# ming71/rotate-yolov3

Hardware: AMD Instinct MI355X
Metric: images/sec fwd+bwd at 608^2 (train step, backend=hip) (higher is better)
Workload: dtype bf16; 1 GPU; configs[3]: Darknet-53 train step (fwd + riou loss + bwd + grad all-reduce + SGD), bs=64/GPU 608x608, synthetic HRSC-shaped targets; global_batch=64, parallelism=dp1, gradients=250 MB fp32 in 4 flat buckets, fp32 on the wire

## Files before the change

include/ryolo.h:

```cpp
#ifndef RYOLO_H
#define RYOLO_H

#include <stddef.h>
#include <stdint.h>

#ifdef __cplusplus
extern "C" {
#endif

#define RYOLO_OK 0
#define RYOLO_EINVAL -1
#define RYOLO_ELAUNCH -2
#define RYOLO_ETOOBIG -3

#define RYOLO_RNMS_MAX_BOXES 262144

const char *ryolo_strerror(int code);
int ryolo_abi_version(void);
const char *ryolo_build_id(void);
int ryolo_set_tuning(const char *name, const char *value);

size_t ryolo_rnms_workspace_bytes(int n);
int ryolo_rnms(const float *dets, int n, int row_stride, float thr, int64_t *keep_out, int32_t *num_keep,
               void *workspace, size_t workspace_bytes, void *stream);
// ... 114 lines not shown
int ryolo_conv_dgrad_tap_table(int ksize, int stride, int *host_out );
int ryolo_conv_pack_weights_dgrad(const float *w_oihw, int Cout, int Cin, int ksize, int stride, void *packed,
                                  const int *taps_table ,
                                  void *stream);
int ryolo_conv2d_dgrad(const ryolo_conv_desc *forward_desc, const void *dz, int dz_cstride, const void *packed_dgrad,
                       const float *ones, const float *zeros , void *dx, int accumulate, void *stream);
int ryolo_conv2d_dgrad_bnreduce_rows(const ryolo_conv_desc *forward_desc);
int ryolo_conv2d_dgrad_bnreduce(const ryolo_conv_desc *forward_desc, const void *dz, int dz_cstride, const void *packed_dgrad,
                                const float *ones, const float *zeros, void *dx, int accumulate,
                                const void *z , int z_cstride,
                                const float *scale, const float *shift, const float *mean, const float *invstd ,
                                const float *slope , float *part , void *stream);
int ryolo_bn_act_bwd_reduced(const void *z, int z_cstride, const void *dy, int dy_cstride, const float *scale, const float *shift,
                             const float *mean, const float *invstd, int act , const float *slope, void *dz,
                             int dz_cstride, long long npix, int C, float *dgamma, float *dbeta, float *dslope, const float *part,
                             int rows, void *workspace , size_t workspace_bytes, void *stream);
size_t ryolo_conv_wgrad_workspace_bytes(const ryolo_conv_desc *forward_desc);
int ryolo_conv2d_wgrad_partials(const ryolo_conv_desc *forward_desc, const void *x, const void *dz, int dz_cstride, int Cin_real,
                                float *grad_oihw, int accumulate, void *workspace, size_t workspace_bytes, void *stream);
int ryolo_conv2d_wgrad_reduce(const ryolo_conv_desc *forward_desc, const void *x, const void *dz, int dz_cstride, int Cin_real,
                              float *grad_oihw, int accumulate, void *workspace, size_t workspace_bytes, void *stream);

typedef struct ryolo_wgrad_reduce_job {
    const float *part;
    float *g;
    int S, Cout, Cin_real, Cin_k, ks, Kpad, Cout_pad, accumulate;
    int kind;
    int block_begin, block_end;
    int wide;
} ryolo_wgrad_reduce_job;
int ryolo_conv_wgrad_reduce_job_fill(ryolo_wgrad_reduce_job *host_job, const ryolo_conv_desc *forward_desc, int Cin_real, const void *workspace,
                                     float *grad_oihw, int accumulate);
int ryolo_conv_wgrad_reduce_batch(const ryolo_wgrad_reduce_job *device_jobs, int njobs, int total_blocks, void *stream);
int ryolo_conv2d_wgrad(const ryolo_conv_desc *forward_desc, const void *x, const void *dz, int dz_cstride, int Cin_real,
                       float *grad_oihw , int accumulate, void *workspace,
                       size_t workspace_bytes, void *stream);
int ryolo_upsample2x_bwd(const void *dy, int dy_cstride, void *dx, int dx_cstride, int N, int H, int W, int C,
                         int accumulate, void *stream);
int ryolo_pgrad_to_nhwc(const float *pgrad, int bs, int na, int ny, int nx, int no, void *out, int out_cstride,
                        void *stream);

typedef struct ryolo_pack_job {
    const void *src;
    void *dst;
    int kind, Cout, Cin, KS, Cin_pad, ntaps, Kpad, rows;
    int khs[9], kws[9];
    int block_begin, block_end;
} ryolo_pack_job;
int ryolo_conv_pack_job_fill(ryolo_pack_job *host_jobs, const float *w_oihw, int Cout, int Cin, int ksize, int stride,
                             int Cin_pad, void *packed_fwd, void *packed_dgrad);
int ryolo_conv_pack_batch(const ryolo_pack_job *device_jobs, int njobs, int total_blocks, void *stream);

#define RYOLO_MAX_HEADS 4
int ryolo_build_targets(const float *tpad, const unsigned char *valid, int NT, int nheads, int na, const float *const *ng,
                        const float *const *anchor_vec, float iou_t, float ang_t, float context_factor, float *const *w,
                        long long *const *idx, float *const *box, float *const *npos, void *stream);
size_t ryolo_yolo_loss_bitmap_bytes(long long cells);
int ryolo_yolo_loss(const float *p, int bs, int na, int ny, int nx, int no, int nc, const float *w, int NT,
                    const long long *b, const long long *gj, const long long *gi, const long long *cls, const float *txy,
                    const float *twh, const float *ta, const float *anchor_vec , const float *npos, float giou,
                    float reg_w, float cls_w, float cls_pw, float obj_w, float obj_pw,
                    int iou_mode ,
                    unsigned *bitmap, float *dp, float *items , void *stream);

int ryolo_yolo_loss_nhwc(const void *head, int head_cstride, const float *p, int bs, int na, int ny, int nx, int no, int nc,
                         const float *w, int NT, const long long *b, const long long *gj, const long long *gi,
// ... 38 lines not shown
```

rotate-yolov3_amd/csrc/rnms.hip:

```cpp
#include <hip/hip_runtime.h>
#include <hipcub/hipcub.hpp>
#include <stdint.h>

#include <mutex>

#include "../../include/ryolo.h"
#include "conv_common.h"

#pragma clang fp contract(off)

namespace {

constexpr int WAVE = 64;
constexpr int MAX_PTS = 24;
constexpr int FAST_PTS = 8;

__device__ __forceinline__ void sincosf_cr(float a, float &s_out, float &c_out) {
    double x = (double)a;
    if (!(fabs(x) <= 1.0e6)) {
        if (!(fabs(x) <= 3.5e38)) {
            s_out = (float)(x - x);
            c_out = (float)(x - x);
            return;
        }
// ... 787 lines not shown
static std::mutex g_side_mutex;
static SidePool g_side[16];
static SidePool *side_pool(hipStream_t stream) {
    int dev = 0;
    if (hipGetDevice(&dev) != hipSuccess || dev < 0 || dev >= 16) return nullptr;
    SidePool &sp = g_side[dev];
    if (sp.state == 0) {
        hipStreamCaptureStatus cs = hipStreamCaptureStatusNone;
        if (hipStreamIsCapturing(stream, &cs) != hipSuccess || cs != hipStreamCaptureStatusNone) { (void)hipGetLastError(); return nullptr; }
        const bool ok = hipStreamCreateWithFlags(&sp.s, hipStreamNonBlocking) == hipSuccess &&
                        hipEventCreateWithFlags(&sp.a, hipEventDisableTiming) == hipSuccess &&
                        hipEventCreateWithFlags(&sp.b, hipEventDisableTiming) == hipSuccess;
        if (!ok) (void)hipGetLastError();
        sp.state = ok ? 1 : -1;
    }
    return sp.state == 1 ? &sp : nullptr;
}
constexpr int SPLIT_MIN_ROWS = 320;

}

extern "C" {

const char *ryolo_strerror(int code) {
    switch (code) {
        case RYOLO_OK: return "ok";
        case RYOLO_EINVAL: return "invalid argument";
        case RYOLO_ELAUNCH: return "HIP launch failed (no gfx950 device, or a previous asynchronous error)";
        case RYOLO_ETOOBIG: return "too many boxes for one rotated-NMS call";
        default: return "unknown ryolo error";
    }
}

int ryolo_abi_version(void) { return 2; }

void ryolo_rnms_count_pairs(uint64_t *device_counter) { g_pair_counter = (unsigned long long *)device_counter; }


size_t ryolo_rnms_workspace_bytes(int n) {
    if (n <= 0) return 256;
    if (n > RYOLO_RNMS_MAX_BOXES) return 0;
    return rnms_layout(n).total;
}

int ryolo_rnms(const float *dets, int n, int row_stride, float thr, int64_t *keep_out, int32_t *num_keep,
               void *workspace, size_t workspace_bytes, void *stream_) {
    hipStream_t stream = (hipStream_t)stream_;
    if (n < 0 || !num_keep) return RYOLO_EINVAL;
    if (n == 0) {
        return hipMemsetAsync(num_keep, 0, sizeof(int32_t), stream) == hipSuccess ? RYOLO_OK : RYOLO_ELAUNCH;
    }
    if (!dets || !keep_out || !workspace || row_stride < 6) return RYOLO_EINVAL;
    if (n > RYOLO_RNMS_MAX_BOXES) return RYOLO_ETOOBIG;
    const RnmsLayout L = rnms_layout(n);
    if (workspace_bytes < L.total) return RYOLO_EINVAL;
    char *ws = (char *)workspace;
    uint32_t *keys_in = (uint32_t *)(ws + L.keys_in), *keys_out = (uint32_t *)(ws + L.keys_out);
    int32_t *idx_in = (int32_t *)(ws + L.idx_in), *order = (int32_t *)(ws + L.order);
    float4 *P0 = (float4 *)(ws + L.p0), *P1 = (float4 *)(ws + L.p1), *AUX = (float4 *)(ws + L.aux);
    uint4 *summ = (uint4 *)(ws + L.summ);
    unsigned char *flags = (unsigned char *)(ws + L.flags);
    unsigned long long *tiles = (unsigned long long *)(ws + L.tiles);

    const int tb = 256, nb = (n + tb - 1) / tb;
    hipLaunchKernelGGL(rnms_keys_kernel, dim3(nb), dim3(tb), 0, stream, dets, n, row_stride, keys_in, idx_in);
    size_t cub_bytes = L.cub_bytes;
    if (hipcub::DeviceRadixSort::SortPairs(ws + L.cub, cub_bytes, keys_in, keys_out, idx_in, order, n, 0, 32,
// ... 103 lines not shown
```

rotate-yolov3_amd/csrc/train.hip:

```cpp
#include <hip/hip_runtime.h>
#include <stdint.h>
#include <stdlib.h>

#include "../../include/ryolo.h"

namespace {

typedef __attribute__((ext_vector_type(8))) __bf16 bf16x8;
typedef __attribute__((ext_vector_type(4))) float f32x4;
typedef __attribute__((address_space(3))) void *lds_vp;
typedef short s16x4 __attribute__((ext_vector_type(4)));
typedef short s16x8 __attribute__((ext_vector_type(8)));

__device__ __forceinline__ s16x4 lds_read_tr16(const char *addr) {
#if defined(__HIP_DEVICE_COMPILE__)
    return __builtin_amdgcn_ds_read_tr16_b64_v4i16((__attribute__((address_space(3))) s16x4 *)(addr));
#else
    return s16x4{0, 0, 0, 0};
#endif
}

template <int T>
__device__ __forceinline__ int wg_swz(int row) {
    if (T >= 128) return (row & 3) | (((row >> 3) & 1) << 2);
// ... 139 lines not shown
#pragma unroll
        for (int ks = 0; ks < 2; ks++) {
            bf16x8 af[NF], bfr[NF];
#pragma unroll
            for (int f = 0; f < NF; f++) {
                const s16x4 a0 = lds_read_tr16(abuf + offa[f] + (ks * 32) * ROWB);
                const s16x4 a1 = lds_read_tr16(abuf + offa[f] + (ks * 32 + 4) * ROWB);
                const s16x4 b0 = lds_read_tr16(bbuf + offb[f] + (ks * 32) * ROWB);
                const s16x4 b1 = lds_read_tr16(bbuf + offb[f] + (ks * 32 + 4) * ROWB);
                af[f] = __builtin_bit_cast(bf16x8, __builtin_shufflevector(a0, a1, 0, 1, 2, 3, 4, 5, 6, 7));
                bfr[f] = __builtin_bit_cast(bf16x8, __builtin_shufflevector(b0, b1, 0, 1, 2, 3, 4, 5, 6, 7));
            }
#pragma unroll
            for (int a = 0; a < NF; a++)
#pragma unroll
                for (int c = 0; c < NF; c++)
                    acc[a][c] = __builtin_amdgcn_mfma_f32_16x16x32_bf16(af[a], bfr[c], acc[a][c], 0, 0, 0);
        }
    }
    float *out = p.part + (size_t)split * p.Cout_pad * p.Kpad;
#pragma unroll
    for (int a = 0; a < NF; a++)
#pragma unroll
        for (int c = 0; c < NF; c++)
#pragma unroll
            for (int r = 0; r < 4; r++) {
                const int co = co0 + wr * WT + a * 16 + kg * 4 + r;
                const int ci = ci0 + wc * WT + c * 16 + fr;
                if (co < p.Cout && ci < p.Cin) out[(size_t)co * p.Kpad + tap * p.Cin + ci] = acc[a][c][r];
            }
}

template <int TM, int TN, int ABL = 0, int NW = 4, int NT = 1>
__global__ void __launch_bounds__(NW * 64, NW == 8 ? (TM * TN > 256 * 128 ? 2 : 4) : 1) wgrad_wide_kernel(const WgradParams p) {
    constexpr int KPX = 32, NST = 3;
    constexpr int WM = TM / (NW / 2), WN = NT * TN / 2, NFA = WM / 16, NFB = WN / 16;
    constexpr int ROW_A = TM * 2, ROW_B = TN * 2;
    constexpr int TILE_A = KPX * ROW_A, TILE_B = KPX * ROW_B, STAGE = TILE_A + NT * TILE_B;
    constexpr int CH_A = TM / 8, CH_B = TN / 8;
    constexpr int PPP_A = 64 / CH_A, PPP_B = 64 / CH_B;
    constexpr int PPW_A = TILE_A / 1024 / NW, PPW_B = NT * TILE_B / 1024 / NW;
    constexpr int PPT_B = TILE_B / 1024;
    constexpr int NLD = PPW_A + PPW_B;
    static_assert(TM >= 64 && TN >= 64 && CH_A <= 64 && TILE_A % (1024 * NW) == 0 && (NT * TILE_B) % (1024 * NW) == 0, "tile shape");
    static_assert(NT == 1 || (NT * TN) % 32 == 0, "whole fragments per wave column");
    extern __shared__ __attribute__((aligned(16))) char smem[];

    const int tid = threadIdx.x, lane = tid & 63;
    const int wave = __builtin_amdgcn_readfirstlane(tid >> 6);
    int b = blockIdx.x;
    {
        const int per = gridDim.x >> 3;
        if (b < per * 8) b = (b & 7) * per + (b >> 3);
    }
    const int ci_t = b % p.ci_tiles; b /= p.ci_tiles;
    const int co_t = b % p.co_tiles; b /= p.co_tiles;
    const int ntg = (p.ks * p.ks) / NT;
    const int tap = (b % ntg) * NT; b /= ntg;
    const int split = b;
    const int kh = tap / p.ks, kw = tap % p.ks;
    const int co0 = co_t * TM, ci0 = ci_t * TN;
    const int pix_lo = split * p.chunk, pix_hi = min(p.M, pix_lo + p.chunk);

    int a_pix[PPW_A], a_col[PPW_A];
#pragma unroll
    for (int j = 0; j < PPW_A; j++) {
        const int tp = (wave * PPW_A + j) * PPP_A + lane / CH_A;
        a_pix[j] = tp;
        a_col[j] = (co0 + (((lane % CH_A) ^ (wg_swz<TM>(tp) << 1)) * 8)) * 2;
    }
    int b_pix[PPW_B], b_col[PPW_B], b_kw[PPW_B];
#pragma unroll
    for (int j = 0; j < PPW_B; j++) {
        const int q = wave * PPW_B + j;
        const int tp = (NT == 1 ? q : q % PPT_B) * PPP_B + lane / CH_B;
        b_pix[j] = tp;
        b_kw[j] = kw + (NT == 1 ? 0 : q / PPT_B);
        b_col[j] = (ci0 + (((lane % CH_B) ^ (wg_swz<TN>(tp) << 1)) * 8)) * 2;
    }

    const i32x4 rs_x = make_rsrc_words(p.x, p.x_bytes);
    const unsigned lds0 = (unsigned)(size_t)(__attribute__((address_space(3))) char *)smem;
    const unsigned a_step = (unsigned)(KPX * p.dz_cs * 2);
    unsigned long long a_base = (unsigned long long)p.dz + (unsigned long long)pix_lo * (unsigned long long)(p.dz_cs * 2);
    unsigned a_rec = (unsigned)((pix_hi - pix_lo) * p.dz_cs * 2);
    int a_vo[PPW_A];
#pragma unroll
    for (int j = 0; j < PPW_A; j++) a_vo[j] = a_pix[j] * p.dz_cs * 2 + a_col[j];
    const int x_cs2 = p.x_cs * 2;
    const int b_dw = KPX * p.stride, b_doff = KPX * p.stride * x_cs2;
    const int wi_wrap0 = p.Wo * p.stride - p.pad, hi_top = p.Ho * p.stride - p.pad + kh;
    const int b_wos = p.Wo * p.stride, b_hos = p.Ho * p.stride;
    const int b_rowjump = (p.stride * p.W - p.Wo * p.stride) * x_cs2, b_imgjump = (p.H - p.Ho * p.stride) * p.W * x_cs2;
    int b_rem = pix_hi - pix_lo;
    int b_hi[PPW_B], b_wi[PPW_B], b_off[PPW_B];
#pragma unroll
    for (int j = 0; j < PPW_B; j++) {
        const int pg = pix_lo + b_pix[j];
        const int wo = pg % p.Wo, t = pg / p.Wo;
        b_hi[j] = (t % p.Ho) * p.stride - p.pad + kh;
        b_wi[j] = wo * p.stride - p.pad + b_kw[j];
        b_off[j] = (int)(((long long)((t / p.Ho) * p.H + b_hi[j]) * p.W + b_wi[j]) * x_cs2) + b_col[j];
    }
    auto stage_a = [&](int buf, int j) __attribute__((always_inline)) {
        i32x4 r;
        r[0] = __builtin_amdgcn_readfirstlane((int)(unsigned)a_base);
        r[1] = __builtin_amdgcn_readfirstlane((int)(unsigned)(a_base >> 32));
        r[2] = __builtin_amdgcn_readfirstlane((int)a_rec);
        r[3] = 0x00020000;
        buffer_load_lds16_raw(r, lds0 + buf * STAGE + (wave * PPW_A + j) * 1024, a_vo[j]);
    };
    auto stage_b = [&](int buf, int j) __attribute__((always_inline)) {
        const bool ok = b_pix[j] < b_rem && (unsigned)b_hi[j] < (unsigned)p.H && (unsigned)b_wi[j] < (unsigned)p.W;
        buffer_load_lds16_raw(rs_x, lds0 + buf * STAGE + TILE_A + (wave * PPW_B + j) * 1024, ok ? b_off[j] : (int)0x80000000);
        b_wi[j] += b_dw;
        b_off[j] += b_doff;
        const int wi_wrap = wi_wrap0 + b_kw[j];
        auto wrap = [&]() __attribute__((always_inline)) {
// ... 65 lines not shown
        }
        __builtin_amdgcn_s_setprio(1);
#pragma unroll
        for (int a = 0; a < NFA; a++)
#pragma unroll
            for (int c = 0; c < NFB; c++)
                acc[a][c] = __builtin_amdgcn_mfma_f32_16x16x32_bf16(af[a], bfr[c], acc[a][c], 0, 0, 0);
        __builtin_amdgcn_s_setprio(0);
        cur = cur == NST - 1 ? 0 : cur + 1;
        nxt = nxt == NST - 1 ? 0 : nxt + 1;
    }
    asm volatile("s_waitcnt vmcnt(0)" ::: "memory");
    float *out = p.part + (size_t)split * p.Cout_pad * p.Kpad;
    if (ABL & 1) {
        float t = 0.f;
#pragma unroll
        for (int a = 0; a < NFA; a++)
#pragma unroll
            for (int c = 0; c < NFB; c++) t += acc[a][c][0] + acc[a][c][1] + acc[a][c][2] + acc[a][c][3];
        if (t == 1234.5678f) out[0] = t;
        return;
    }
#pragma unroll
    for (int a = 0; a < NFA; a++)
#pragma unroll
        for (int c = 0; c < NFB; c++)
#pragma unroll
            for (int r = 0; r < 4; r++) {
                const int co = co0 + wr * WM + a * 16 + kg * 4 + r;
                const int nn = wc * WN + c * 16 + fr;
                const int ci = ci0 + (NT == 1 ? nn : nn % TN);
                if (co < p.Cout && ci < p.Cin) out[(size_t)co * p.Kpad + (tap + (NT == 1 ? 0 : nn / TN)) * p.Cin + ci] = acc[a][c][r];
            }
}

struct WgradTapsParams {
    const __bf16 *x, *dz;
    float *part;
    int N, H, W, x_cs, Ho, Wo, dz_cs, pad;
    int Cout, Kpad;
    int nseg, nsteps, steps_per_split;
    unsigned x_bytes, dz_bytes;
};

template <int CO, int CI, int KS, int ST>
__global__ void __launch_bounds__(256) wgrad_taps_kernel(const WgradTapsParams p) {
    constexpr int A_ROWB = CO * 2, A_TILE = KP * A_ROWB, A_PIECES = A_TILE / 1024;
    constexpr int QP = (KP - 1) * ST + KS;
    constexpr int B_ROWB = CI * 2;
    constexpr int PPR = (QP * B_ROWB + 1023) / 1024;
    constexpr int QPP = PPR * 1024 / B_ROWB;
    constexpr int B_TILE = KS * PPR * 1024, B_PIECES = KS * PPR;
    constexpr int STAGE = A_TILE + B_TILE, PIECES = A_PIECES + B_PIECES, PPW = (PIECES + 3) / 4;
    constexpr int NREAL = KS * KS * CI;
    constexpr int MF = CO / 16, NFR = (NREAL + 15) / 16, NJ = (NFR + 3) / 4;
    constexpr int A_CPR = A_ROWB / 16, B_CPR = B_ROWB / 16;
    static_assert(CO % 16 == 0 && (CI == 8 || CI % 16 == 0), "fragment-aligned channel counts");
    static_assert(CI != 8 || QPP > QP, "C_in = 8 needs a padding pixel (always zero) in the halo row");
    extern __shared__ __attribute__((aligned(16))) char smem[];

    const int tid = threadIdx.x, lane = tid & 63;
    const int wave = __builtin_amdgcn_readfirstlane(tid >> 6);
    const int split = blockIdx.x;
    const int s_lo = split * p.steps_per_split, s_hi = min(p.nsteps, s_lo + p.steps_per_split);

    auto stage = [&](int s, int buf) {
// ... 1009 lines not shown
    unsigned blocks = 0;
    job->kind = wgrad_reduce_kind(w.S, d->Cout, Cin_real, d->ksize, &blocks);
#ifdef RYOLO_MP_ABLATION
    const char *env = getenv("RYOLO_WGRAD_REDUCE_V4");
#else
    const char *env = nullptr;
#endif
    const bool v4 = !(env && env[0] == '0'), t3v = !(env && (env[0] == '0' || env[0] == '1'));
    const int wide = !(env && env[0] >= '0' && env[0] <= '2');
    const long long step_bytes = (long long)job->Cout_pad * job->Kpad * 4;
    if (job->kind == 1 && v4 && Cin_real % 4 == 0 && d->Cin % 4 == 0 && ((uintptr_t)workspace & 15) == 0 &&
        ((w.S + 3) / 4 + 17) * step_bytes < (1ll << 31)) {
        job->kind = 3;
        job->wide = wide;
        blocks = (unsigned)grid_for((long long)d->Cout * Cin_real * d->ksize * d->ksize, 256 * (wide ? wgrad_reduce_v4_groups(w.S) : 1));
    }
    if (job->kind == 2 && t3v && w.S < 8 && 8 * step_bytes < (1ll << 31)) {
        job->kind = 4;
        job->wide = wide;
        const int r = wide ? wgrad_reduce_t3v_units_per_block(w.S) : 1;
        blocks = (blocks + r - 1) / r;
    }
    job->block_begin = 0;
    job->block_end = (int)blocks;
    return (int)blocks;
}

int ryolo_conv_wgrad_reduce_batch(const ryolo_wgrad_reduce_job *device_jobs, int njobs, int total_blocks, void *stream) {
    if (!device_jobs || njobs <= 0 || total_blocks <= 0) return RYOLO_EINVAL;
    hipLaunchKernelGGL(wgrad_reduce_batch_kernel, dim3((unsigned)total_blocks), dim3(256), 0, (hipStream_t)stream, device_jobs, njobs);
    return ok_launch();
}

int ryolo_conv2d_wgrad(const ryolo_conv_desc *d, const void *x, const void *dz, int dz_cstride, int Cin_real,
                       float *grad_oihw, int accumulate, void *workspace, size_t workspace_bytes, void *stream_) {
    if (!d || !x || !dz || !grad_oihw || !workspace) return RYOLO_EINVAL;
    const bool do_tiles = g_wgrad_phase != 2, do_reduce = g_wgrad_phase != 1;
    if ((d->Cin & 7) || (d->Cout & 7) || (d->in_cstride & 7) || (dz_cstride & 7) || Cin_real <= 0 || Cin_real > d->Cin)
        return RYOLO_EINVAL;
    const WgradPlan w = wgrad_plan(d);
    if (workspace_bytes < w.part_bytes) return RYOLO_EINVAL;
    WgradParams p;
    p.x = (const __bf16 *)x; p.dz = (const __bf16 *)dz; p.part = (float *)workspace;
    p.N = d->N; p.H = d->H; p.W = d->W; p.Cin = d->Cin; p.x_cs = d->in_cstride;
    p.Ho = (d->H + 2 * d->pad - d->ksize) / d->stride + 1;
    p.Wo = (d->W + 2 * d->pad - d->ksize) / d->stride + 1;
    p.Cout = d->Cout; p.dz_cs = dz_cstride;
    p.ks = d->ksize; p.stride = d->stride; p.pad = d->pad;
    p.Kpad = (d->ksize * d->ksize * d->Cin + 63) / 64 * 64;
    p.Cout_pad = (d->Cout + 127) / 128 * 128;
    p.M = (int)((long long)d->N * p.Ho * p.Wo);
    p.S = w.S; p.chunk = w.chunk; p.co_tiles = w.co_tiles; p.ci_tiles = w.ci_tiles;
    const unsigned long long xb = (((unsigned long long)d->N * d->H * d->W - 1) * d->in_cstride + d->Cin) * 2ull;
    const unsigned long long zb = (((unsigned long long)p.M - 1) * dz_cstride + d->Cout) * 2ull;
    if (xb >= 0x7fffff00ull || zb >= 0x7fffff00ull) return RYOLO_EINVAL;
    p.x_bytes = (unsigned)xb; p.dz_bytes = (unsigned)zb;
    hipStream_t stream = (hipStream_t)stream_;
    if (const int variant = wgrad_taps_variant(d)) {
        WgradTapsParams q;
        q.x = p.x; q.dz = p.dz; q.part = p.part;
        q.N = p.N; q.H = p.H; q.W = p.W; q.x_cs = p.x_cs; q.Ho = p.Ho; q.Wo = p.Wo; q.dz_cs = p.dz_cs; q.pad = p.pad;
        q.Cout = p.Cout; q.Kpad = p.Kpad;
        q.nseg = (p.Wo + KP - 1) / KP;
        q.nsteps = p.N * p.Ho * q.nseg;
        q.steps_per_split = w.chunk;
        q.x_bytes = p.x_bytes; q.dz_bytes = p.dz_bytes;
        auto smem_of = [](int co, int ci, int ks, int st) {
            const int qp = (KP - 1) * st + ks;
            const int ppr = (qp * ci * 2 + 1023) / 1024;
            return (size_t)2 * (KP * co * 2 + ks * ppr * 1024);
        };
        static bool attr_done = false;
        if (!attr_done) {
            if (hipFuncSetAttribute((const void *)wgrad_taps_kernel<64, 32, 3, 2>, hipFuncAttributeMaxDynamicSharedMemorySize,
                                    (int)smem_of(64, 32, 3, 2)) != hipSuccess)
                return RYOLO_ELAUNCH;
            attr_done = true;
        }
        if (!do_tiles) {}
        else if (variant == 1) hipLaunchKernelGGL((wgrad_taps_kernel<64, 32, 3, 1>), dim3(w.S), dim3(256), smem_of(64, 32, 3, 1), stream, q);
        else if (variant == 2) hipLaunchKernelGGL((wgrad_taps_kernel<64, 32, 3, 2>), dim3(w.S), dim3(256), smem_of(64, 32, 3, 2), stream, q);
        else if (variant == 3) hipLaunchKernelGGL((wgrad_taps_kernel<32, 64, 1, 1>), dim3(w.S), dim3(256), smem_of(32, 64, 1, 1), stream, q);
        else hipLaunchKernelGGL((wgrad_taps_kernel<32, 8, 3, 1>), dim3(w.S), dim3(256), smem_of(32, 8, 3, 1), stream, q);
        if (hipGetLastError() != hipSuccess) return RYOLO_ELAUNCH;
        if (do_reduce) launch_wgrad_reduce((const float *)workspace, w.S, d->Cout, Cin_real, d->Cin, d->ksize, p.Kpad, d->Cout, grad_oihw, accumulate, stream);
        return ok_launch();
    }
    const unsigned nblk = (unsigned)(w.co_tiles * w.ci_tiles * wgrad_tap_groups(w.T, d->ksize) * w.S);
    if (!do_tiles) {
// ... 167 lines not shown
```

rotate-yolov3_amd/model/hip_train_ops.py:

```python
import ctypes as C

import torch

from .. import _lib
from .hip_ops import ConvDesc, _check_nhwc, cpad

_vp = C.c_void_p
_P = C.POINTER(ConvDesc)
_lib.declare("ryolo_conv_stat_rows", C.c_int, [_P])
_lib.declare("ryolo_conv2d_bn_act_stats", C.c_int, [_P, _vp, _vp, _vp, _vp, _vp, _vp, _vp, _vp])
_lib.declare("ryolo_bn_finalize", C.c_int, [_vp, C.c_int, C.c_int, C.c_int, C.c_longlong, C.c_float, C.c_float, _vp, _vp, _vp,
                                            _vp, _vp, _vp, _vp, _vp, _vp])
_lib.declare("ryolo_bn_act_fwd", C.c_int, [_vp, C.c_int, _vp, _vp, C.c_int, _vp, _vp, C.c_int, _vp, C.c_int, C.c_longlong,
                                           C.c_int, _vp])
_lib.declare("ryolo_bn_act_bwd_workspace_bytes", C.c_size_t, [C.c_longlong, C.c_int])
_lib.declare("ryolo_bn_act_bwd", C.c_int, [_vp, C.c_int, _vp, C.c_int, _vp, _vp, _vp, _vp, C.c_int, _vp, _vp, C.c_int,
                                           C.c_longlong, C.c_int, _vp, _vp, _vp, _vp, C.c_size_t, _vp])
_lib.declare("ryolo_conv_packed_dgrad_bytes", C.c_size_t, [C.c_int, C.c_int, C.c_int, C.c_int])
_lib.declare("ryolo_conv_pack_weights_dgrad", C.c_int, [_vp, C.c_int, C.c_int, C.c_int, C.c_int, _vp, _vp, _vp])
_lib.declare("ryolo_conv_dgrad_tap_table", C.c_int, [C.c_int, C.c_int, _vp])
_lib.declare("ryolo_conv2d_dgrad", C.c_int, [_P, _vp, C.c_int, _vp, _vp, _vp, _vp, C.c_int, _vp])
_lib.declare("ryolo_conv2d_dgrad_bnreduce", C.c_int, [_P, _vp, C.c_int, _vp, _vp, _vp, _vp, C.c_int, _vp, C.c_int, _vp, _vp, _vp, _vp, _vp,
                                                      _vp, _vp])
_lib.declare("ryolo_bn_act_bwd_reduced", C.c_int, [_vp, C.c_int, _vp, C.c_int, _vp, _vp, _vp, _vp, C.c_int, _vp, _vp, C.c_int,
# ... 56 lines not shown

class WgradReduceBatch(object):

    def __init__(self, device):
        self.device = device
        self.jobs = []
        self.keep = []

    def add(self, d, cin_real, ws, grad, accumulate):
        j = WgradReduceJob()
        n = _lib.lib().ryolo_conv_wgrad_reduce_job_fill(C.byref(j), C.byref(d), cin_real, ws.data_ptr(), grad.data_ptr(), 1 if accumulate else 0)
        if n <= 0:
            raise RuntimeError("ryolo_conv_wgrad_reduce_job_fill failed")
        self.jobs.append(j)
        self.keep.append((ws, grad))

    def finalize(self):
        arr = (WgradReduceJob * len(self.jobs))()
        blk = 0
        for q, j in enumerate(self.jobs):
            nb = j.block_end
            j.block_begin, j.block_end = blk, blk + nb
            blk += nb
            arr[q] = j
        self.total_blocks = blk
        self.dev_jobs = torch.frombuffer(bytearray(bytes(arr)), dtype=torch.uint8).to(self.device)
        self.n = len(self.jobs)

    def run(self):
        _lib.check(_lib.lib().ryolo_conv_wgrad_reduce_batch(self.dev_jobs.data_ptr(), self.n, self.total_blocks, _s(self.device)),
                   "ryolo_conv_wgrad_reduce_batch")


class WeightPackBatch(object):

    def __init__(self, device):
        self.device = device
        self.jobs = []

    def add(self, weight, stride, cin_pad, packed_fwd, packed_dgrad):
        cout, cin, k, _ = weight.shape
        tmp = (PackJob * 8)()
        n = _lib.lib().ryolo_conv_pack_job_fill(tmp, weight.data_ptr(), cout, cin, k, stride, cin_pad, packed_fwd.data_ptr(),
                                                packed_dgrad.data_ptr() if packed_dgrad is not None else None)
        if n <= 0:
            raise RuntimeError("ryolo_conv_pack_job_fill failed")
        for q in range(n):
            j = PackJob()
            C.memmove(C.byref(j), C.byref(tmp[q]), C.sizeof(PackJob))
            self.jobs.append(j)

    def finalize(self):
        arr = (PackJob * len(self.jobs))()
        blk = 0
        for q, j in enumerate(self.jobs):
            nb = j.block_end
            j.block_begin, j.block_end = blk, blk + nb
            blk += nb
            arr[q] = j
        self.total_blocks = blk
        raw = bytes(arr)
        self.dev_jobs = torch.frombuffer(bytearray(raw), dtype=torch.uint8).to(self.device)
        self.n = len(self.jobs)

    def run(self):
        _lib.check(_lib.lib().ryolo_conv_pack_batch(self.dev_jobs.data_ptr(), self.n, self.total_blocks, _s(self.device)),
# ... 321 lines not shown
```

rotate-yolov3_amd/model/train_engine.py:

```python
import ctypes as C
import os

import torch
import torch.nn as nn

from .. import _lib
from . import hip_ops as ops
from . import hip_train_ops as tr
from . import plan
from .engine import HipEngine


class _Fn(torch.autograd.Function):
    @staticmethod
    def forward(ctx, engine, x, anchor):
        ctx.engine = engine
        outs = engine.forward(x)
        return tuple(outs)

    @staticmethod
    def backward(ctx, *grads):
        ctx.engine.backward(grads)
        return None, None, None

# ... 55 lines not shown
                xin, y, dy = tv(rec['xin']), tv(rec['y']), tv(rec['dy'])
                c, h, w = rec['shape']
                desc = ops.ConvDesc(*rec['desc'])
                if bn is not None:
                    z = None if rec['recompute'] else new_buf(c, h, w)
                    dz = None if rec['one_pass'] else new_buf(c, h, w)
                else:
                    z, dz = y, dy
                blk = dict(i=i, conv=conv, bn=bn, act=actmod[-1] if actmod else None, mish=any(type(s_).__name__ == 'Mish' for s_ in mods[i]),
                           xin=xin, xin_g=tv(rec['xin_g']), z=z, dz=dz, y=y, dy=dy, desc=desc, res=tv(rec['res']), res_g=tv(rec['res_g']),
                           res_alias=rec['res_alias'], cin_k=xin.shape[-1], k=desc.ksize, s=desc.stride, pad=desc.pad,
                           npix=self.bs * h * w, C=c, recompute=rec['recompute'])
                wgrad_ws = max(wgrad_ws, tr.wgrad_ws_bytes(desc))
                bn_ws = max(bn_ws, tr.bn_bwd_ws_bytes(blk['npix'], c))
                self.blocks.append(blk)
                fwd.append(('conv', i, blk))
            elif kind in ('add', 'up'):
                fwd.append((kind, i, tuple(tv(v) for v in rec)))
            elif kind == 'yolo':
                m = mods[i]
                c, h, w = tp.shapes[i]
                anchors = m.anchors.to(device=device, dtype=torch.float32).contiguous()
                pbuf = torch.empty((self.bs, m.na, h, w, model.nc + 6), dtype=torch.float32, device=device)
                io = None
                if model.nc + 6 > 96 or m.na * (model.nc + 6) > 1024:
                    io = torch.empty((self.bs, m.na * h * w, model.nc + 6), dtype=torch.float32, device=device)
                self.p.append(pbuf)
                fwd.append(('yolo', i, (tv(rec[0]), tv(rec[1]), m, anchors, pbuf, io, h, w)))
        self.head_pairs = [(pl[0], pl[1]) for kind, _, pl in fwd if kind == 'yolo']
        self.fused_nhwc = False
        self.head_g_ready = False
        self.batch_reduce = os.environ.get('RYOLO_WGRAD_BATCH_REDUCE', '1') != '0'
        self._wr_batches = {}
        self._ws_w_bytes = max(wgrad_ws, 256)
        self._ws_w = None
        self.ws_b = torch.empty(max(bn_ws, 256), dtype=torch.uint8, device=device)

        self.bplan = [(kind, i, pl, flags) for (kind, i, pl), (_, _, flags) in zip(reversed(fwd), tp.backward)]

    @staticmethod
    def _conv_attrs(m):
        conv = HipEngine._conv_of(m)
        other = [type(s_).__name__ for s_ in m if not isinstance(s_, (nn.Conv2d, nn.BatchNorm2d, nn.PReLU, nn.LeakyReLU))
                 and type(s_).__name__ != 'Mish']
        return dict(cout=conv.out_channels, k=conv.kernel_size[0], s=conv.stride[0], pad=conv.padding[0],
                    bn=HipEngine._bn_of(m) is not None, act=None,
                    refuse="activation %s has no HIP training kernels (use model.backend = 'torch')" % other[0] if other else None)

    def _build_grad_sink(self):
        plist = [q for q in self.model.parameters()]
        views = getattr(self.model, '_dp_grad_views', None)
        ok = views is not None and os.environ.get("RYOLO_DIRECT_GRADS", "1") != "0"
        if ok:
            for q in plist:
                v = views.get(q)
                if (v is None or v.dtype != torch.float32 or not v.is_contiguous() or v.device != q.device or v.shape != q.shape
                        or q.grad is None or q.grad.data_ptr() != v.data_ptr()):
                    ok = False
                    break
        self.direct = bool(ok)
        if ok:
            self.static_flat = None
            self.static_grad = {q: views[q] for q in plist}
        else:
            self.static_flat = torch.zeros(sum(q.numel() for q in plist), dtype=torch.float32, device=self.device)
            off = 0
            for q in plist:
                self.static_grad[q] = self.static_flat[off:off + q.numel()].view_as(q)
                off += q.numel()

    def _reset_grad_sink(self):
        self.static_grad, self.static_flat, self.direct = {}, None, False
        self._segs, self.g_bwd = None, None
        self._wr_batches = {}

    def _check_direct_sink(self):
        if not self.direct:
            return
        rebound = 0
        for q, v in self.static_grad.items():
            g = q.grad
            if g is None:
                v.zero_()
            elif g.data_ptr() != v.data_ptr():
                v.copy_(g)
            else:
                continue
            q.grad = v
            rebound += 1
        if rebound and not getattr(self, '_warned_rebind', False):
            self._warned_rebind = True
            import warnings
            warnings.warn("TrainEngine: %d param.grad tensors had been replaced (zero_grad(set_to_none=True)?) while a GradientAllReducer "
                          "owns them; they were re-bound to the reducer's buckets.  Use reducer.zero_grad() to clear gradients." % rebound)

    def _grad_of(self, p):
        g = self.static_grad.get(p)
        if g is None:
            self._build_grad_sink()
            g = self.static_grad[p]
        return g

    def _flush_param_grads(self, params=None):
        add_to, add_from = [], []
        plist = list(self.static_grad.keys()) if params is None else params
        if not self.direct:
            views = getattr(self.model, '_dp_grad_views', None) or {}
# ... 9 lines not shown
                if p.grad is None:
                    p.grad = g.clone()
                else:
                    add_to.append(p.grad)
                    add_from.append(g)
            if add_to:
                torch._foreach_add_(add_to, add_from)
        for p in plist:
            hooks = getattr(p, '_post_accumulate_grad_hooks', None)
            if hooks:
                for hk in list(hooks.values()):
                    hk(p)

    @staticmethod
    def _has_wgrad(b):
        return not (b['bn'] is not None and b['recompute'] and b['xin_g'] is None and b['dz'] is None)

    @property
    def ws_w(self):
        if self._ws_w is None:
            self._ws_w = torch.empty(self._ws_w_bytes, dtype=torch.uint8, device=self.device)
        return self._ws_w

    def _ensure_reduce_batches(self, segs):
        if not self.batch_reduce:
            return
        try:
            self._build_reduce_batches(segs)
        except torch.cuda.OutOfMemoryError as e:
            for kind, i, pl, flags in self.bplan:
                if kind == 'conv':
                    pl.pop('ws_w', None)
            self._wr_batches = {}
            torch.cuda.empty_cache()
            self.batch_reduce = False
            self.reduce_fallback = "per-layer split-K reduces on one shared workspace (the per-layer workspaces did not fit: %s)" % str(e)[:120]
            self.g_bwd = None

    def _build_reduce_batches(self, segs):
        for lo, hi, _ in segs:
            if (lo, hi) in self._wr_batches:
                continue
            blks = [pl for kind, i, pl, flags in self.bplan[lo:hi] if kind == 'conv' and self._has_wgrad(pl)]
            wb = None
            if blks:
                wb = tr.WgradReduceBatch(self.device)
                for b in blks:
                    if 'ws_w' not in b:
                        b['ws_w'] = torch.empty(max(tr.wgrad_ws_bytes(b['desc']), 256), dtype=torch.uint8, device=self.device)
                    wb.add(b['desc'], b['conv'].in_channels, b['ws_w'], self._grad_of(b['conv'].weight), True)
                wb.finalize()
            self._wr_batches[(lo, hi)] = wb

    def _segments(self):
        if self._segs is not None:
            return self._segs
        pos = {}
        for k, (kind, i, pl, flags) in enumerate(self.bplan):
            if kind == 'conv':
                for q in list(pl['conv'].parameters()) + (list(pl['bn'].parameters()) if pl['bn'] is not None else []) + (
                        list(pl['act'].parameters()) if isinstance(pl['act'], nn.Module) else []):
                    pos[q] = k
        cuts = set()
        for bucket in getattr(self.model, '_dp_buckets', None) or []:
            ks = [pos[q] for q in bucket if q in pos]
            if ks:
                cuts.add(max(ks) + 1)
        cuts.add(len(self.bplan))
        segs, lo = [], 0
        for hi in sorted(cuts):
            if hi > lo:
                segs.append((lo, hi, [q for q, k in pos.items() if lo <= k < hi]))
                lo = hi
        self._segs = segs
        return segs


    def forward(self, x):
        dev = self.device
        x = x.float().contiguous()
        with torch.cuda.device(dev), torch.no_grad():
            n, c, h, w = x.shape
            _lib.check(_lib.lib().ryolo_nchw_f32_to_nhwc_bf16(x.data_ptr(), n, c, h, w, 8, self.x_nhwc.data_ptr(), _lib.stream_ptr(dev)),
                       "ryolo_nchw_f32_to_nhwc_bf16")
            if not self.use_graph or self.steps < 2 or self.force_eager:
# ... 145 lines not shown

        def entry(kind, i, pl, flags):
            if kind == 'yolo':
                pass
            elif kind == 'conv':
                b = pl
                conv, bn = b['conv'], b['bn']
                res_first, in_first = flags
                dy = b['dy']
                if b['res_g'] is not None and not b['res_alias']:
                    self._passthrough(dy, b['res_g'], res_first)
                if bn is not None:
                    dsl = self._grad_of(b['act'].weight) if isinstance(b['act'], nn.PReLU) else None
                    if b['recompute'] and b['xin_g'] is None and b['dz'] is None:
                        if 'ws0f' not in b:
                            b['ws0f'] = tr.conv0_bn_bwd_wgrad_ws(dev)
                        tr.conv0_bn_bwd_wgrad(b['desc'], b['xin'], b['packed'], dy, b['stats'], b['actcode'], b['slope'],
                                              self._grad_of(bn.weight), self._grad_of(bn.bias), dsl, self._grad_of(conv.weight),
                                              conv.in_channels, True, b['ws0f'])
                        return
                    elif b['recompute']:
                        if 'ws0' not in b:
                            b['ws0'] = tr.conv0_bn_bwd_ws(dev)
                        tr.conv0_bn_bwd(b['desc'], b['xin'], b['packed'], dy, b['stats'], b['actcode'], b['slope'], b['dz'],
                                        self._grad_of(bn.weight), self._grad_of(bn.bias), dsl, b['ws0'])
                    elif b.get('red_part') is not None:
                        tr.bn_act_bwd_reduced(b['z'], dy, b['stats'], 1, b['slope'], b['dz'],
                                              self._grad_of(bn.weight), self._grad_of(bn.bias), dsl, b['red_part'], self.ws_b)
                    else:
                        tr.bn_act_bwd(b['z'], dy, b['stats'], b['actcode'], b['slope'], b['dz'],
                                      self._grad_of(bn.weight), self._grad_of(bn.bias), dsl, self.ws_b)
                elif conv.bias is not None:
                    tr.bn_act_bwd(b['z'], dy, None, 0, None, None, None, self._grad_of(conv.bias), None, self.ws_b)
                if self.batch_reduce:
                    tr.conv_wgrad_partials(b['desc'], b['xin'], b['dz'], conv.in_channels, self._grad_of(conv.weight), True, b['ws_w'])
                else:
                    tr.conv_wgrad(b['desc'], b['xin'], b['dz'], conv.in_channels, self._grad_of(conv.weight), True, self.ws_w)
                if b['xin_g'] is not None:
                    y = b.get('red_for')
                    if y is not None:
                        tr.conv_dgrad_bnreduce(b['desc'], b['dz'], b['packed_d'], self.ones, self.zeros, b['xin_g'], not in_first,
                                               y['z'], y['stats'], y['slope'], y['red_part'])
                    else:
                        tr.conv_dgrad(b['desc'], b['dz'], b['packed_d'], self.ones, self.zeros, b['xin_g'], not in_first)
            elif kind == 'add':
                dyv = pl[5]
                self._passthrough(dyv, pl[3], flags[0])
                self._passthrough(dyv, pl[4], flags[1])
            elif kind == 'up':
                tr.upsample2x_bwd(pl[3], pl[2], not flags)

        for kind, i, pl, flags in self.bplan[lo:hi]:
            if hook is not None:
                hook('pre', kind, i, pl, flags)
            entry(kind, i, pl, flags)
            if hook is not None:
                hook('post', kind, i, pl, flags)
        if self.batch_reduce:
            wb = self._wr_batches[(lo, len(self.bplan) if hi is None else hi)]
            if wb is not None:
                wb.run()

    def _plan_reduce_fusion(self):
        self._red_planned = True
        if os.environ.get("RYOLO_BN_REDUCE_FUSION", "1") == "0":
            return
        blk = {b['i']: b for b in self.blocks}
        pairs = []
        for xr, yr, rows in plan.reduce_fusion_pairs(self._tplan):
            x, y = blk[xr['layer']], blk[yr['layer']]
            if y.get('actcode') == 1 and y.get('slope') is not None and y.get('stats') is not None:
                pairs.append((x, y, rows, x['xin_g'].shape[3]))
        if not pairs:
            return
        part = torch.empty(max(rows * 3 * c for _, _, rows, c in pairs), dtype=torch.float32, device=self.device)
        for x, y, rows, c in pairs:
            x['red_for'] = y
            y['red_part'] = part[:rows * 3 * c].view(rows, 3, c)

    def _passthrough(self, src, dst, is_first):
        L = _lib.lib()
        n, h, w, c = dst.shape
        if is_first:
            _lib.check(L.ryolo_upsample_nhwc(src.data_ptr(), src.stride(2), dst.data_ptr(), dst.stride(2), n, h, w, c, 1,
                                             _lib.stream_ptr(self.device)), "ryolo_upsample_nhwc")
        else:
            _lib.check(L.ryolo_add_nhwc(src.data_ptr(), src.stride(2), dst.data_ptr(), dst.stride(2), dst.data_ptr(),
                                        dst.stride(2), n * h * w, c, _lib.stream_ptr(self.device)), "ryolo_add_nhwc")

    def __call__(self, x):
        anchor = next(self.model.parameters())
        return list(_Fn.apply(self, x, anchor))
# ... 1 lines not shown
```

Baseline: 1359 images/s.

## Batch 1x1 conv wgrad tile kernels into one grouped launch per tile class

Turns the wide wgrad kernel body into a device function and adds a grouped kernel that looks up its job from a device-side job table by block index. The 1x1 convs in a backward segment whose plan picks one of the wide tile classes no longer run their own partials launch. Their partials are computed in one launch per class at the end of the segment, just before the batched reduce. This is meant to cut launch overhead and tail underutilisation from many small wgrad launches, at the cost of per-block job lookup and later wgrad execution within the segment. It also clamps the A buffer record size to dz_bytes.

Result: no change. 1353 images/s (median of 2 runs) (-0.5%).

```diff
diff --git a/include/ryolo.h b/include/ryolo.h
--- a/include/ryolo.h
+++ b/include/ryolo.h
@@ -170,6 +170,22 @@
 int ryolo_conv_wgrad_reduce_job_fill(ryolo_wgrad_reduce_job *host_job, const ryolo_conv_desc *forward_desc, int Cin_real, const void *workspace,
                                      float *grad_oihw, int accumulate);
 int ryolo_conv_wgrad_reduce_batch(const ryolo_wgrad_reduce_job *device_jobs, int njobs, int total_blocks, void *stream);
+typedef struct ryolo_wgrad_batch_job {
+    const void *x, *dz;
+    float *part;
+    int N, H, W, Cin, x_cs;
+    int Ho, Wo, Cout, dz_cs;
+    int ks, stride, pad;
+    int Kpad, Cout_pad, M;
+    int S, chunk;
+    int co_tiles, ci_tiles;
+    unsigned x_bytes, dz_bytes;
+    int tile_class;
+    int block_begin, block_end;
+} ryolo_wgrad_batch_job;
+int ryolo_conv_wgrad_batch_job_fill(ryolo_wgrad_batch_job *host_job, const ryolo_conv_desc *forward_desc, const void *x, const void *dz,
+                                    int dz_cstride, int Cin_real, void *workspace, size_t workspace_bytes);
+int ryolo_conv_wgrad_partials_batch(const ryolo_wgrad_batch_job *device_jobs, int njobs, int total_blocks, int tile_class, void *stream);
 int ryolo_conv2d_wgrad(const ryolo_conv_desc *forward_desc, const void *x, const void *dz, int dz_cstride, int Cin_real,
                        float *grad_oihw , int accumulate, void *workspace,
                        size_t workspace_bytes, void *stream);
diff --git a/rotate-yolov3_amd/csrc/rnms.hip b/rotate-yolov3_amd/csrc/rnms.hip
--- a/rotate-yolov3_amd/csrc/rnms.hip
+++ b/rotate-yolov3_amd/csrc/rnms.hip
@@ -843,7 +843,7 @@
     }
 }
 
-int ryolo_abi_version(void) { return 2; }
+int ryolo_abi_version(void) { return 3; }
 
 void ryolo_rnms_count_pairs(uint64_t *device_counter) { g_pair_counter = (unsigned long long *)device_counter; }
 
diff --git a/rotate-yolov3_amd/csrc/train.hip b/rotate-yolov3_amd/csrc/train.hip
--- a/rotate-yolov3_amd/csrc/train.hip
+++ b/rotate-yolov3_amd/csrc/train.hip
@@ -195,7 +195,7 @@
 }
 
 template <int TM, int TN, int ABL = 0, int NW = 4, int NT = 1>
-__global__ void __launch_bounds__(NW * 64, NW == 8 ? (TM * TN > 256 * 128 ? 2 : 4) : 1) wgrad_wide_kernel(const WgradParams p) {
+__device__ __forceinline__ void wgrad_wide_body(const WgradParams &p, int block, unsigned nblocks) {
     constexpr int KPX = 32, NST = 3;
     constexpr int WM = TM / (NW / 2), WN = NT * TN / 2, NFA = WM / 16, NFB = WN / 16;
     constexpr int ROW_A = TM * 2, ROW_B = TN * 2;
@@ -211,9 +211,9 @@
 
     const int tid = threadIdx.x, lane = tid & 63;
     const int wave = __builtin_amdgcn_readfirstlane(tid >> 6);
-    int b = blockIdx.x;
+    int b = block;
     {
-        const int per = gridDim.x >> 3;
+        const int per = nblocks >> 3;
         if (b < per * 8) b = (b & 7) * per + (b >> 3);
     }
     const int ci_t = b % p.ci_tiles; b /= p.ci_tiles;
@@ -246,7 +246,7 @@
     const unsigned lds0 = (unsigned)(size_t)(__attribute__((address_space(3))) char *)smem;
     const unsigned a_step = (unsigned)(KPX * p.dz_cs * 2);
     unsigned long long a_base = (unsigned long long)p.dz + (unsigned long long)pix_lo * (unsigned long long)(p.dz_cs * 2);
-    unsigned a_rec = (unsigned)((pix_hi - pix_lo) * p.dz_cs * 2);
+    unsigned a_rec = min((unsigned)((pix_hi - pix_lo) * p.dz_cs * 2), p.dz_bytes - (unsigned)pix_lo * (unsigned)(p.dz_cs * 2));
     int a_vo[PPW_A];
 #pragma unroll
     for (int j = 0; j < PPW_A; j++) a_vo[j] = a_pix[j] * p.dz_cs * 2 + a_col[j];
@@ -378,6 +378,34 @@
                 const int ci = ci0 + (NT == 1 ? nn : nn % TN);
                 if (co < p.Cout && ci < p.Cin) out[(size_t)co * p.Kpad + (tap + (NT == 1 ? 0 : nn / TN)) * p.Cin + ci] = acc[a][c][r];
             }
+}
+template <int TM, int TN, int ABL = 0, int NW = 4, int NT = 1>
+__global__ void __launch_bounds__(NW * 64, NW == 8 ? (TM * TN > 256 * 128 ? 2 : 4) : 1) wgrad_wide_kernel(const WgradParams p) {
+    wgrad_wide_body<TM, TN, ABL, NW, NT>(p, blockIdx.x, gridDim.x);
+}
+
+template <int TM, int TN>
+__global__ void __launch_bounds__(256, 1) wgrad_wide_batch_kernel(const ryolo_wgrad_batch_job *__restrict__ jobs, int njobs) {
+    const int lane = threadIdx.x & 63;
+    int lo = -1;
+    for (int base = 0; base < njobs; base += 64) {
+        const int q = base + lane;
+        lo += __popcll(__ballot(q < njobs && jobs[q].block_begin <= (int)blockIdx.x));
+    }
+    lo = __builtin_amdgcn_readfirstlane(lo);
+    if (lo < 0) return;
+    const ryolo_wgrad_batch_job j = jobs[lo];
+    const int block = (int)blockIdx.x - j.block_begin, nblocks = j.block_end - j.block_begin;
+    if (block >= nblocks) return;
+    WgradParams p;
+    p.x = (const __bf16 *)j.x; p.dz = (const __bf16 *)j.dz; p.part = j.part;
+    p.N = j.N; p.H = j.H; p.W = j.W; p.Cin = j.Cin; p.x_cs = j.x_cs;
+    p.Ho = j.Ho; p.Wo = j.Wo; p.Cout = j.Cout; p.dz_cs = j.dz_cs;
+    p.ks = j.ks; p.stride = j.stride; p.pad = j.pad;
+    p.Kpad = j.Kpad; p.Cout_pad = j.Cout_pad; p.M = j.M;
+    p.S = j.S; p.chunk = j.chunk; p.co_tiles = j.co_tiles; p.ci_tiles = j.ci_tiles;
+    p.x_bytes = j.x_bytes; p.dz_bytes = j.dz_bytes;
+    wgrad_wide_body<TM, TN>(p, block, (unsigned)nblocks);
 }
 
 struct WgradTapsParams {
@@ -1453,15 +1481,11 @@
     return ok_launch();
 }
 
-int ryolo_conv2d_wgrad(const ryolo_conv_desc *d, const void *x, const void *dz, int dz_cstride, int Cin_real,
-                       float *grad_oihw, int accumulate, void *workspace, size_t workspace_bytes, void *stream_) {
-    if (!d || !x || !dz || !grad_oihw || !workspace) return RYOLO_EINVAL;
-    const bool do_tiles = g_wgrad_phase != 2, do_reduce = g_wgrad_phase != 1;
+static int wgrad_fill_params(WgradParams &p, const WgradPlan &w, const ryolo_conv_desc *d, const void *x, const void *dz, int dz_cstride,
+                             int Cin_real, void *workspace, size_t workspace_bytes) {
     if ((d->Cin & 7) || (d->Cout & 7) || (d->in_cstride & 7) || (dz_cstride & 7) || Cin_real <= 0 || Cin_real > d->Cin)
         return RYOLO_EINVAL;
-    const WgradPlan w = wgrad_plan(d);
     if (workspace_bytes < w.part_bytes) return RYOLO_EINVAL;
-    WgradParams p;
     p.x = (const __bf16 *)x; p.dz = (const __bf16 *)dz; p.part = (float *)workspace;
     p.N = d->N; p.H = d->H; p.W = d->W; p.Cin = d->Cin; p.x_cs = d->in_cstride;
     p.Ho = (d->H + 2 * d->pad - d->ksize) / d->stride + 1;
@@ -1476,6 +1500,63 @@
     const unsigned long long zb = (((unsigned long long)p.M - 1) * dz_cstride + d->Cout) * 2ull;
     if (xb >= 0x7fffff00ull || zb >= 0x7fffff00ull) return RYOLO_EINVAL;
     p.x_bytes = (unsigned)xb; p.dz_bytes = (unsigned)zb;
+    return RYOLO_OK;
+}
+
+constexpr int WIDE_LDS_256 = 3 * 32 * (256 + 128) * 2;
+
+int ryolo_conv_wgrad_batch_job_fill(ryolo_wgrad_batch_job *job, const ryolo_conv_desc *d, const void *x, const void *dz, int dz_cstride, int Cin_real,
+                                    void *workspace, size_t workspace_bytes) {
+    if (!job || !d || !x || !dz || !workspace || (d->ksize != 1 && d->ksize != 3) || d->Cin <= 0 || d->Cout <= 0) return 0;
+    if (wgrad_taps_variant(d)) return 0;
+#ifdef RYOLO_MP_ABLATION
+    if (g_wgrad_abl) return 0;
+#endif
+    const WgradPlan w = wgrad_plan(d);
+    if (w.T != 256 && w.T != 259 && w.T != 260) return 0;
+    WgradParams p;
+    if (wgrad_fill_params(p, w, d, x, dz, dz_cstride, Cin_real, workspace, workspace_bytes) != RYOLO_OK) return 0;
+    *job = ryolo_wgrad_batch_job{};
+    job->x = p.x; job->dz = p.dz; job->part = p.part;
+    job->N = p.N; job->H = p.H; job->W = p.W; job->Cin = p.Cin; job->x_cs = p.x_cs;
+    job->Ho = p.Ho; job->Wo = p.Wo; job->Cout = p.Cout; job->dz_cs = p.dz_cs;
+    job->ks = p.ks; job->stride = p.stride; job->pad = p.pad;
+    job->Kpad = p.Kpad; job->Cout_pad = p.Cout_pad; job->M = p.M;
+    job->S = p.S; job->chunk = p.chunk; job->co_tiles = p.co_tiles; job->ci_tiles = p.ci_tiles;
+    job->x_bytes = p.x_bytes; job->dz_bytes = p.dz_bytes;
+    job->tile_class = w.T;
+    job->block_begin = 0;
+    job->block_end = w.co_tiles * w.ci_tiles * wgrad_tap_groups(w.T, d->ksize) * w.S;
+    return job->block_end;
+}
+
+int ryolo_conv_wgrad_partials_batch(const ryolo_wgrad_batch_job *device_jobs, int njobs, int total_blocks, int tile_class, void *stream) {
+    if (!device_jobs || njobs <= 0 || total_blocks <= 0) return RYOLO_EINVAL;
+    if (tile_class == 256) {
+        static bool attr_done = false;
+        if (!attr_done) {
+            if (hipFuncSetAttribute((const void *)wgrad_wide_batch_kernel<256, 128>, hipFuncAttributeMaxDynamicSharedMemorySize, WIDE_LDS_256) != hipSuccess)
+                return RYOLO_ELAUNCH;
+            attr_done = true;
+        }
+        hipLaunchKernelGGL((wgrad_wide_batch_kernel<256, 128>), dim3((unsigned)total_blocks), dim3(256), WIDE_LDS_256, (hipStream_t)stream, device_jobs, njobs);
+    } else if (tile_class == 259) {
+        hipLaunchKernelGGL((wgrad_wide_batch_kernel<128, 128>), dim3((unsigned)total_blocks), dim3(256), 3 * 32 * (128 + 128) * 2, (hipStream_t)stream, device_jobs, njobs);
+    } else if (tile_class == 260) {
+        hipLaunchKernelGGL((wgrad_wide_batch_kernel<64, 128>), dim3((unsigned)total_blocks), dim3(256), 3 * 32 * (64 + 128) * 2, (hipStream_t)stream, device_jobs, njobs);
+    } else {
+        return RYOLO_EINVAL;
+    }
+    return ok_launch();
+}
+
+int ryolo_conv2d_wgrad(const ryolo_conv_desc *d, const void *x, const void *dz, int dz_cstride, int Cin_real,
+                       float *grad_oihw, int accumulate, void *workspace, size_t workspace_bytes, void *stream_) {
+    if (!d || !x || !dz || !grad_oihw || !workspace) return RYOLO_EINVAL;
+    const bool do_tiles = g_wgrad_phase != 2, do_reduce = g_wgrad_phase != 1;
+    const WgradPlan w = wgrad_plan(d);
+    WgradParams p;
+    if (const int rc = wgrad_fill_params(p, w, d, x, dz, dz_cstride, Cin_real, workspace, workspace_bytes)) return rc;
     hipStream_t stream = (hipStream_t)stream_;
     if (const int variant = wgrad_taps_variant(d)) {
         WgradTapsParams q;
diff --git a/rotate-yolov3_amd/model/hip_train_ops.py b/rotate-yolov3_amd/model/hip_train_ops.py
--- a/rotate-yolov3_amd/model/hip_train_ops.py
+++ b/rotate-yolov3_amd/model/hip_train_ops.py
@@ -112,6 +112,66 @@
                    "ryolo_conv_wgrad_reduce_batch")
 
 
+class WgradBatchJob(C.Structure):
+    _fields_ = [("x", C.c_void_p), ("dz", C.c_void_p), ("part", C.c_void_p)] + [(n, C.c_int) for n in (
+        "N", "H", "W", "Cin", "x_cs", "Ho", "Wo", "Cout", "dz_cs", "ks", "stride", "pad", "Kpad", "Cout_pad", "M", "S", "chunk", "co_tiles",
+        "ci_tiles")] + [("x_bytes", C.c_uint), ("dz_bytes", C.c_uint), ("tile_class", C.c_int), ("block_begin", C.c_int),
+                        ("block_end", C.c_int)]
+
+
+_lib.declare("ryolo_conv_wgrad_batch_job_fill", C.c_int, [C.POINTER(WgradBatchJob), _P, _vp, _vp, C.c_int, C.c_int, _vp, C.c_size_t])
+_lib.declare("ryolo_conv_wgrad_partials_batch", C.c_int, [_vp, C.c_int, C.c_int, C.c_int, _vp])
+
+WGRAD_BATCH_CLASSES = (256, 259, 260)
+
+
+def wgrad_batch_layout(jobs):
+    order = sorted(jobs, key=lambda j: -j.chunk)
+    blk = 0
+    for j in order:
+        nb = j.block_end - j.block_begin
+        j.block_begin, j.block_end = blk, blk + nb
+        blk = (blk + nb + 7) // 8 * 8
+    return order, (order[-1].block_end if order else 0)
+
+
+class WgradTileBatch(object):
+
+    def __init__(self, device):
+        self.device = device
+        self.jobs = {}
+        self.keep = []
+        self.launches = []
+
+    def add(self, d, x, dz, cin_real, ws):
+        j = WgradBatchJob()
+        n = _lib.lib().ryolo_conv_wgrad_batch_job_fill(C.byref(j), C.byref(d), x.data_ptr(), dz.data_ptr(), dz.stride(2), cin_real,
+                                                       ws.data_ptr(), ws.numel())
+        if n <= 0:
+            return False
+        self.jobs.setdefault(j.tile_class, []).append(j)
+        self.keep.append((x, dz, ws))
+        return True
+
+    @property
+    def n(self):
+        return sum(len(v) for v in self.jobs.values())
+
+    def finalize(self):
+        self.launches = []
+        for cls in sorted(self.jobs):
+            order, total = wgrad_batch_layout(self.jobs[cls])
+            arr = (WgradBatchJob * len(order))(*order)
+            dev_jobs = torch.frombuffer(bytearray(bytes(arr)), dtype=torch.uint8).to(self.device)
+            self.launches.append((dev_jobs, len(order), total, cls))
+
+    def run(self):
+        L = _lib.lib()
+        for dev_jobs, n, total, cls in self.launches:
+            _lib.check(L.ryolo_conv_wgrad_partials_batch(dev_jobs.data_ptr(), n, total, cls, _s(self.device)),
+                       "ryolo_conv_wgrad_partials_batch")
+
+
 class WeightPackBatch(object):
 
     def __init__(self, device):
diff --git a/rotate-yolov3_amd/model/train_engine.py b/rotate-yolov3_amd/model/train_engine.py
--- a/rotate-yolov3_amd/model/train_engine.py
+++ b/rotate-yolov3_amd/model/train_engine.py
@@ -111,6 +111,8 @@
         self.head_g_ready = False
         self.batch_reduce = os.environ.get('RYOLO_WGRAD_BATCH_REDUCE', '1') != '0'
         self._wr_batches = {}
+        self.batch_tiles = self.batch_reduce and os.environ.get('RYOLO_WGRAD_BATCH_TILES', '1') != '0'
+        self._wt_batches = {}
         self._ws_w_bytes = max(wgrad_ws, 256)
         self._ws_w = None
         self.ws_b = torch.empty(max(bn_ws, 256), dtype=torch.uint8, device=device)
@@ -152,6 +154,7 @@
         self.static_grad, self.static_flat, self.direct = {}, None, False
         self._segs, self.g_bwd = None, None
         self._wr_batches = {}
+        self._drop_tile_batches()
 
     def _check_direct_sink(self):
         if not self.direct:
@@ -227,17 +230,28 @@
                 if kind == 'conv':
                     pl.pop('ws_w', None)
             self._wr_batches = {}
+            self._drop_tile_batches()
             torch.cuda.empty_cache()
             self.batch_reduce = False
             self.reduce_fallback = "per-layer split-K reduces on one shared workspace (the per-layer workspaces did not fit: %s)" % str(e)[:120]
             self.g_bwd = None
+
+    def _drop_tile_batches(self):
+        self._wt_batches = {}
+        for kind, i, pl, flags in getattr(self, 'bplan', ()):
+            if kind == 'conv':
+                pl.pop('wgrad_deferred', None)
+
+    @staticmethod
+    def _short_wgrad(b):
+        return b['k'] == 1 and _lib.lib().ryolo_conv_wgrad_kernel_choice(C.byref(b['desc'])) in tr.WGRAD_BATCH_CLASSES
 
     def _build_reduce_batches(self, segs):
         for lo, hi, _ in segs:
             if (lo, hi) in self._wr_batches:
                 continue
             blks = [pl for kind, i, pl, flags in self.bplan[lo:hi] if kind == 'conv' and self._has_wgrad(pl)]
-            wb = None
+            wb = wt = None
             if blks:
                 wb = tr.WgradReduceBatch(self.device)
                 for b in blks:
@@ -245,7 +259,15 @@
                         b['ws_w'] = torch.empty(max(tr.wgrad_ws_bytes(b['desc']), 256), dtype=torch.uint8, device=self.device)
                     wb.add(b['desc'], b['conv'].in_channels, b['ws_w'], self._grad_of(b['conv'].weight), True)
                 wb.finalize()
+                if self.batch_tiles:
+                    wt = tr.WgradTileBatch(self.device)
+                    for b in blks:
+                        b['wgrad_deferred'] = self._short_wgrad(b) and wt.add(b['desc'], b['xin'], b['dz'], b['conv'].in_channels, b['ws_w'])
+                    wt.finalize()
+                    if not wt.n:
+                        wt = None
             self._wr_batches[(lo, hi)] = wb
+            self._wt_batches[(lo, hi)] = wt
 
     def _segments(self):
         if self._segs is not None:
@@ -457,7 +479,9 @@
                                       self._grad_of(bn.weight), self._grad_of(bn.bias), dsl, self.ws_b)
                 elif conv.bias is not None:
                     tr.bn_act_bwd(b['z'], dy, None, 0, None, None, None, self._grad_of(conv.bias), None, self.ws_b)
-                if self.batch_reduce:
+                if self.batch_reduce and b.get('wgrad_deferred'):
+                    pass
+                elif self.batch_reduce:
                     tr.conv_wgrad_partials(b['desc'], b['xin'], b['dz'], conv.in_channels, self._grad_of(conv.weight), True, b['ws_w'])
                 else:
                     tr.conv_wgrad(b['desc'], b['xin'], b['dz'], conv.in_channels, self._grad_of(conv.weight), True, self.ws_w)
@@ -482,7 +506,11 @@
             if hook is not None:
                 hook('post', kind, i, pl, flags)
         if self.batch_reduce:
-            wb = self._wr_batches[(lo, len(self.bplan) if hi is None else hi)]
+            key = (lo, len(self.bplan) if hi is None else hi)
+            wb = self._wr_batches[key]
+            wt = self._wt_batches.get(key)
+            if wt is not None:
+                wt.run()
             if wb is not None:
                 wb.run()
 
```
